# hmorimitsu/ptlflow

Measured on NVIDIA H100. Metric: frame-pairs/sec RAFT 1024x436 12-iter, higher is better.
Workload: dtype f16 storage, f32 accumulate/coordinates

## Files before the change

include/ptlflow_b200.h:

```cpp
#ifndef PTLFLOW_B200_H_
#define PTLFLOW_B200_H_

#include <stddef.h>
#include <stdint.h>

#ifdef __cplusplus
extern "C" {
#endif

#if defined(__GNUC__)
#define PFB_API __attribute__((visibility("default")))
#else
#define PFB_API
#endif

typedef void* pfb_stream;

typedef enum { PFB_F32 = 0, PFB_F16 = 1, PFB_BF16 = 2 } pfb_dtype;

typedef enum {
  PFB_OK = 0,
  PFB_ERR_ARG = -1,
  PFB_ERR_CUDA = -2,
  PFB_ERR_UNSUPPORTED = -3
// ... 54 lines not shown
  PFB_EPI_LINEAR = 0,
  PFB_EPI_RELU = 1,
  PFB_EPI_GRU_ZR = 2,
  PFB_EPI_GRU_Q = 3,
  PFB_EPI_FLOW = 4,
  PFB_EPI_RELU_APPEND_FLOW = 5,
  PFB_EPI_AXPY = 6,
  PFB_EPI_LINEAR_F32 = 7,
  PFB_EPI_GELU = 8,
  PFB_EPI_RESIDUAL_GELU = 9,
  PFB_EPI_LINEAR_APPEND_FLOW = 10
} pfb_epilogue;

typedef struct {
  const void* ptr;
  int channels;
  int stride;
  int offset;
  int is_f32;
} pfb_conv_src;

typedef struct {
  pfb_conv_src src[PFB_MAX_SRC];
  int nsrc;
  int B, H, W;
  int KH, KW;
  int Cout;
  int Cout_pad;
  const void* weight;
  const float* bias;
  int epilogue;
  float scale;
  void* out;
  int out_stride, out_offset;
  const void* aux_h;
  void* aux_z;
  int hidden;
  float* coords;
  const float* flow;
  pfb_dtype dtype;
  int impl;
  const void* weight_k;
  int Cin_pad, Cout_pad_k;
  const void* addend;
  int addend_stride;
  int w_rows_per_sample;
  const void* residual;
  int residual_stride, residual_offset;
  const float* post_w;
  const float* post_b;
} pfb_conv_params;

PFB_API int pfb_conv2d(const pfb_conv_params* p, pfb_stream stream);

PFB_API int pfb_pack_conv_weight(const void* src, void* dst, int Cout, int Cin, int KH, int KW, int Cout_pad,
                         int col_offset, pfb_dtype src_dtype, pfb_dtype dst_dtype, pfb_stream stream);
PFB_API int pfb_pack_bias(const void* src, float* dst, int n, int offset, pfb_dtype src_dtype, pfb_stream stream);
PFB_API int pfb_pack_conv_weight_kmajor(const void* src, void* dst, int Cout, int Cin, int KH, int KW, int Cout_pad_k,
                                        int row_offset, const int* src_channels, int nsrc, int Cin_pad,
                                        pfb_dtype src_dtype, pfb_dtype dst_dtype, pfb_stream stream);

PFB_API int pfb_depthwise_conv_gelu(const void* x, int in_stride, int in_offset, void* out, int out_stride, int out_offset,
                                    const float* weight, const float* bias, int B, int H, int W, int C, int k, pfb_dtype dtype,
                                    pfb_stream stream);

PFB_API int pfb_depthwise_conv_layernorm(const void* x, int in_stride, int in_offset, void* out, int out_stride, int out_offset,
                                         const float* weight, const float* bias, int B, int H, int W, int C, int k, float eps,
                                         pfb_dtype dtype, pfb_stream stream);

PFB_API int pfb_convex_upsample(const float* coords, const void* mask, float* out, float* flow_small, int B, int H,
                        int W, int out_h, int out_w, int pad_top, int pad_left, pfb_dtype dtype,
                        pfb_stream stream);
PFB_API int pfb_upflow8(const float* coords, float* out, float* flow_small, int B, int H, int W, int out_h, int out_w,
                int pad_top, int pad_left, pfb_stream stream);

PFB_API int pfb_softmax_rows(void* x, size_t rows, int cols, pfb_dtype dtype, pfb_stream stream);
PFB_API int pfb_attention_softmax_relpos(const void* logits, const float* th, const float* tw, size_t table_stride, void* attn,
                                         size_t rows, int H, int W, int P, pfb_dtype dtype, pfb_stream stream);
PFB_API int pfb_transpose_pm(const void* in, void* out, int B, int HW, int C, int HW_pad, pfb_dtype dtype, pfb_stream stream);

PFB_API int pfb_flow_tap_gather(const float* taps, int tstride, const float* bias, float* coords, float* flow, int B, int H, int W,
                                pfb_stream stream);

PFB_API int pfb_context_split(const void* cnet, void* net, void* inp, int B, int H, int W, int hidden, int context,
                      pfb_dtype dtype, pfb_stream stream);
PFB_API int pfb_init_coords(float* coords, const float* flow_init_nchw, int B, int H, int W, pfb_stream stream);
PFB_API int pfb_forward_interpolate(const float* flow_nchw, float* out_nchw, int B, int H, int W, pfb_stream stream);

typedef enum {
  PFB_L_CONVC1 = 0, PFB_L_CONVC2, PFB_L_CONVF1, PFB_L_CONVF2, PFB_L_CONV,
  PFB_L_GRU_ZR1, PFB_L_GRU_Q1, PFB_L_GRU_ZR2, PFB_L_GRU_Q2,
  PFB_L_FLOW1, PFB_L_FLOW2, PFB_L_MASK1, PFB_L_MASK2,
  PFB_L_AGG_V,
  PFB_L_FLOW2T,
  PFB_L_CTX_ZR1, PFB_L_CTX_Q1, PFB_L_CTX_ZR2, PFB_L_CTX_Q2,
  PFB_L_GRUX_ZR1, PFB_L_GRUX_Q1, PFB_L_GRUX_ZR2, PFB_L_GRUX_Q2,
  PFB_L_CONVC2F2,
  PFB_L_AGG_PROJ,
  PFB_L_COUNT
} pfb_layer_id;

typedef struct {
  const void* weight;
  const float* bias;
  int Cout, Cout_pad, Cin, KH, KW;
  const void* weight_k;
// ... 196 lines not shown
```

ptlflow_b200/_lib.py:

```python
from __future__ import annotations

import ctypes as C
import threading
import os
from typing import Optional

import torch

_PKG = os.path.dirname(os.path.abspath(__file__))
LIB_PATH = os.path.join(_PKG, "lib", "libptlflow_b200.so")

PFB_MAX_LEVELS = 8
PFB_MAX_SRC = 4

F32, F16, BF16 = 0, 1, 2
_DTYPES = {torch.float32: F32, torch.float16: F16, torch.bfloat16: BF16}

EPI_LINEAR, EPI_RELU, EPI_GRU_ZR, EPI_GRU_Q, EPI_FLOW, EPI_RELU_APPEND_FLOW, EPI_AXPY, EPI_LINEAR_F32 = range(8)
EPI_GELU, EPI_RESIDUAL_GELU, EPI_LINEAR_APPEND_FLOW = range(8, 11)
ENC_CONV_LINEAR, ENC_CONV_BIAS_RELU, ENC_CONV_BIAS_RELU_RESIDUAL = range(3)

(L_CONVC1, L_CONVC2, L_CONVF1, L_CONVF2, L_CONV, L_GRU_ZR1, L_GRU_Q1, L_GRU_ZR2, L_GRU_Q2,
 L_FLOW1, L_FLOW2, L_MASK1, L_MASK2, L_AGG_V, L_FLOW2T,
 L_CTX_ZR1, L_CTX_Q1, L_CTX_ZR2, L_CTX_Q2, L_GRUX_ZR1, L_GRUX_Q1, L_GRUX_ZR2, L_GRUX_Q2, L_CONVC2F2, L_AGG_PROJ, L_COUNT) = range(26)
# ... 65 lines not shown
    _fields_ = [("blocks", PcBlock * SK_BLOCKS), ("convf1", Layer), ("mask1", Layer), ("mask2", Layer),
                ("agg_v", Layer), ("agg_proj", Layer)]


PFB_SR_MAX_BLOCKS = 8


class ConvNextBlock(C.Structure):
    _fields_ = [("dw_k", C.c_int), ("dw_weight", C.c_void_p), ("dw_bias", C.c_void_p), ("pw1", Layer), ("out", Layer)]


class SearaftWeights(C.Structure):
    _fields_ = [("init_conv", Layer), ("convc1", Layer), ("convc2", Layer), ("convf1", Layer), ("convf2", Layer), ("conv", Layer),
                ("num_blocks", C.c_int), ("blocks", ConvNextBlock * PFB_SR_MAX_BLOCKS), ("ln_eps", C.c_float),
                ("flow1", Layer), ("flow2", Layer), ("flow2t", Layer), ("mask1", Layer), ("mask2", Layer)]


class XcitBlock(C.Structure):
    _fields_ = [("pos_proj", Layer), ("qk", Layer), ("v_weight", C.c_void_p), ("v_bias", C.c_void_p), ("proj_weight", C.c_void_p),
                ("proj_bias", C.c_void_p), ("temperature", C.c_void_p), ("ln3_weight", C.c_void_p), ("ln3_bias", C.c_void_p),
                ("dw1_weight", C.c_void_p), ("dw1_bias", C.c_void_p), ("gn_weight", C.c_void_p), ("gn_bias", C.c_void_p),
                ("dw2_weight", C.c_void_p), ("dw2_bias", C.c_void_p), ("fc1", Layer), ("fc2", Layer), ("ln_eps", C.c_float),
                ("gn_eps", C.c_float)]


class CcmrWeights(C.Structure):
    _fields_ = [("raft", RaftWeights), ("context", XcitBlock), ("aggregator", XcitBlock)]


_lib: Optional[C.CDLL] = None

_I, _P, _S = C.c_int, C.c_void_p, C.c_void_p
_PP = C.POINTER(C.c_void_p)
SIGNATURES = {
    "pfb_version": (_I, []),
    "pfb_last_error": (C.c_char_p, []),
    "pfb_device_arch": (_I, []),
    "pfb_stream_create": (_I, [_PP]),
    "pfb_stream_destroy": (_I, [_S]),
    "pfb_corr_volume_build": (_I, [_P, _P, _PP, _I, _I, _I, _I, _I, _I, _I, _S]),
    "pfb_corr_volume_build_ex": (_I, [_P, _P, _PP, _I, _I, _I, _I, _I, _I, _I, C.c_float, _I, _I, _S]),
    "pfb_corr_level_bytes": (C.c_size_t, [_I, _I, _I, _I, _I]),
    "pfb_corr_lookup": (_I, [_PP, _P, _P, _I, _I, _I, _I, _I, _I, _I, _I, _I, _S]),
    "pfb_corr_lookup_ex": (_I, [_PP, C.POINTER(C.c_int), C.POINTER(C.c_int), _P, _P, _I, _I, _I, _I, _I, _I, _I, _I, _I, _S]),
    "pfb_corr_level_bytes_tiled": (C.c_size_t, [_I, _I, _I, _I, _I, _I]),
    "pfb_corr_volume_build_tiled": (_I, [_P, _P, _PP, _I, _I, _I, _I, _I, _I, _I, C.c_float, _I, _S]),
    "pfb_corr_lookup_tiled": (_I, [_PP, _P, _P, _I, _I, _I, _I, _I, _I, _I, _I, _I, _S]),
    "pfb_corr_lookup_onthefly": (_I, [_P, _PP, _P, _P, _I, _I, _I, _I, _I, _I, _I, _I, _I, _I, _S]),
    "pfb_corr_lookup_onthefly_tc_workspace_bytes": (C.c_size_t, [_I, _I, _I]),
    "pfb_corr_lookup_onthefly_tc": (_I, [_P, _PP, _P, _P, _P, _I, _I, _I, _I, _I, _I, _I, _I, _S]),
    "pfb_alt_corr_forward": (_I, [_P, _P, _P, _P, _I, _I, _I, _I, _I, _I, _I, _I, _I, _S]),
    "pfb_avg_pool2x2_nhwc": (_I, [_P, _P, _I, _I, _I, _I, _I, _S]),
    "pfb_conv2d": (_I, [C.POINTER(ConvParams), _S]),
    "pfb_pack_conv_weight": (_I, [_P, _P, _I, _I, _I, _I, _I, _I, _I, _I, _S]),
    "pfb_pack_bias": (_I, [_P, _P, _I, _I, _I, _S]),
    "pfb_pack_conv_weight_kmajor": (_I, [_P, _P, _I, _I, _I, _I, _I, _I, C.POINTER(C.c_int), _I, _I, _I, _I, _S]),
    "pfb_convex_upsample": (_I, [_P, _P, _P, _P, _I, _I, _I, _I, _I, _I, _I, _I, _S]),
    "pfb_upflow8": (_I, [_P, _P, _P, _I, _I, _I, _I, _I, _I, _I, _S]),
    "pfb_softmax_rows": (_I, [_P, C.c_size_t, _I, _I, _S]),
    "pfb_attention_softmax_relpos": (_I, [_P, _P, _P, C.c_size_t, _P, C.c_size_t, _I, _I, _I, _I, _S]),
    "pfb_transpose_pm": (_I, [_P, _P, _I, _I, _I, _I, _I, _S]),
    "pfb_flow_tap_gather": (_I, [_P, _I, _P, _P, _P, _I, _I, _I, _S]),
    "pfb_context_split": (_I, [_P, _P, _P, _I, _I, _I, _I, _I, _I, _S]),
    "pfb_init_coords": (_I, [_P, _P, _I, _I, _I, _S]),
    "pfb_forward_interpolate": (_I, [_P, _P, _I, _I, _I, _S]),
    "pfb_raft_workspace_bytes": (C.c_size_t, [C.POINTER(RaftCfg)]),
    "pfb_raft_refine": (_I, [C.POINTER(RaftCfg), C.POINTER(RaftWeights), C.POINTER(RaftBuffers), _S]),
    "pfb_preprocess_frames": (_I, [_P, _P, _I, _I, _I, _I, _I, _I, _I, _I, _I, _S]),
    "pfb_instance_norm_workspace_bytes": (C.c_size_t, [_I, _I]),
    "pfb_instance_norm_act": (_I, [_P, _P, _P, _P, _I, _I, _I, _I, C.c_float, _I, _I, _S]),
    "pfb_instance_norm_apply": (_I, [_P, _P, _P, _P, _I, _I, _I, _I, C.c_float, _I, _I, _S]),
    "pfb_flow_conv7x7": (_I, [_P, _P, _P, _P, _I, _I, _I, _I, _I, _I, _S]),
    "pfb_first_conv7x7s2": (_I, [_P, _P, _P, _P, _P, _I, _I, _I, _I, _I, _S]),
    "pfb_bias_act": (_I, [_P, _P, _P, _P, _P, _I, _I, _I, _I, _I, _I, _S]),
    "pfb_enc_conv3x3_supported": (_I, [_I, _I, _I]),
    "pfb_enc_conv3x3": (_I, [_P, _P, _P, _P, _P, _I, _I, _I, _I, _I, _I, _I, _I, _I, _S]),
    "pfb_launch_count": (C.c_ulonglong, [_I]),
    "pfb_profile_enable": (_I, [_I]),
    "pfb_profile_collect": (_I, [C.POINTER(C.c_double), C.POINTER(C.c_ulonglong), _I]),
    "pfb_raft_update_iter": (_I, [C.POINTER(RaftCfg), C.POINTER(RaftWeights), C.POINTER(RaftBuffers), _P, _P, _S]),
    "pfb_depthwise_conv_gelu": (_I, [_P, _I, _I, _P, _I, _I, _P, _P, _I, _I, _I, _I, _I, _I, _S]),
    "pfb_skflow_workspace_bytes": (C.c_size_t, [C.POINTER(RaftCfg)]),
    "pfb_skflow_refine": (_I, [C.POINTER(RaftCfg), C.POINTER(SkflowWeights), C.POINTER(RaftBuffers), _S]),
    "pfb_skflow_update_iter": (_I, [C.POINTER(RaftCfg), C.POINTER(SkflowWeights), C.POINTER(RaftBuffers), _P, _P, _S]),
    "pfb_depthwise_conv_layernorm": (_I, [_P, _I, _I, _P, _I, _I, _P, _P, _I, _I, _I, _I, _I, C.c_float, _I, _S]),
    "pfb_searaft_workspace_bytes": (C.c_size_t, [C.POINTER(RaftCfg)]),
    "pfb_searaft_refine": (_I, [C.POINTER(RaftCfg), C.POINTER(SearaftWeights), C.POINTER(RaftBuffers), _S]),
    "pfb_searaft_update_iter": (_I, [C.POINTER(RaftCfg), C.POINTER(SearaftWeights), C.POINTER(RaftBuffers), _P, _P, _S]),
    "pfb_corr_lookup_onthefly_ex": (_I, [_P, _PP, _P, _P, _I, _I, _I, _I, _I, _I, C.c_float, _I, _I, _I, _I, _S]),
    "pfb_corr_lookup_onthefly_tc_ex": (_I, [_P, _PP, _P, _P, _P, _I, _I, _I, _I, _I, _I, C.c_float, _I, _I, _S]),
    "pfb_group_norm_act": (_I, [_P, _P, _P, _P, _P, _P, _P, _I, _I, _I, _I, _I, C.c_float, _I, _I, _S]),
    "pfb_group_norm_apply": (_I, [_P, _P, _P, _P, _P, _P, _P, _I, _I, _I, _I, _I, C.c_float, _I, _I, _S]),
    "pfb_upsample2x_concat": (_I, [_P, _I, _P, _I, _P, _I, _I, _I, _I, _S]),
    "pfb_convex_upsample2x": (_I, [_P, _P, _P, _I, _I, _I, _I, _I, _I, _I, _I, _I, _S]),
    "pfb_downflow": (_I, [_P, _P, _I, _I, _I, _I, _I, _S]),
    "pfb_msraft_workspace_bytes": (C.c_size_t, [C.POINTER(RaftCfg)]),
    "pfb_msraft_refine": (_I, [C.POINTER(RaftCfg), C.POINTER(RaftWeights), C.POINTER(RaftBuffers), C.c_float, _P, _S]),
    "pfb_msraft_update_iter": (_I, [C.POINTER(RaftCfg), C.POINTER(RaftWeights), C.POINTER(RaftBuffers), _P, _P, C.c_float, _S]),
    "pfb_layernorm": (_I, [_P, _I, _I, _P, _I, _I, _P, _P, C.c_size_t, _I, C.c_float, _I, _S]),
    "pfb_depthwise_conv3x3_ex": (_I, [_P, _I, _I, _P, _I, _I, _P, _P, _P, _I, _I, _I, _I, _I, _I, _I, _I, _S]),
    "pfb_fourier_features": (_I, [_P, _I, _I, _I, _S]),
    "pfb_xca_stats_workspace_bytes": (C.c_size_t, [_I, _I]),
    "pfb_xca_stats": (_I, [_P, _I, _I, _I, _I, _I, _P, _P, _I, _S]),
    "pfb_xca_fold": (_I, [_P, _P, _P, _P, _P, _P, _P, _P, _P, _I, _I, _S]),
    "pfb_convex_handover2x": (_I, [_P, _P, _P, _I, _I, _I, _I, _S]),
    "pfb_upflow2": (_I, [_P, _P, _I, _I, _I, _I, _I, _I, _I, _S]),
# ... 96 lines not shown
```

ptlflow_b200/csrc/common.cuh:

```cuda
#pragma once
#include <cuda_bf16.h>
#include <cuda_fp16.h>
#include <cuda_runtime.h>
#include <stdint.h>
#include <stdio.h>

#include "../../include/ptlflow_b200.h"

namespace pfb {

void set_error(const char* fmt, ...);

#define PFB_CHECK_ARG(cond, ...)           \
  do {                                     \
    if (!(cond)) {                         \
      ::pfb::set_error(__VA_ARGS__);       \
      return PFB_ERR_ARG;                  \
    }                                      \
  } while (0)

#define PFB_CUDA(call)                                                                        \
  do {                                                                                        \
    cudaError_t e__ = (call);                                                                 \
    if (e__ != cudaSuccess) {                                                                 \
// ... 31 lines not shown
  else if (dt == PFB_F16) reinterpret_cast<__half*>(p)[i] = __float2half_rn(v);
  else reinterpret_cast<__nv_bfloat16*>(p)[i] = __float2bfloat16_rn(v);
}

__device__ __forceinline__ float sigmoid_f32(float x) { return 1.0f / (1.0f + expf(-x)); }
__device__ __forceinline__ float gelu_f32(float x) { return 0.5f * x * (1.0f + erff(x * 0.70710678118654752f)); }

#define PFB_DISPATCH_DTYPE(dt, T, ...)                        \
  do {                                                        \
    if ((dt) == PFB_F32) { using T = float; __VA_ARGS__; }    \
    else if ((dt) == PFB_F16) { using T = __half; __VA_ARGS__; } \
    else { using T = __nv_bfloat16; __VA_ARGS__; }            \
  } while (0)

inline int ceil_div(int a, int b) { return (a + b - 1) / b; }
inline size_t ceil_div_sz(size_t a, size_t b) { return (a + b - 1) / b; }
inline size_t align_up(size_t a, size_t b) { return (a + b - 1) / b * b; }

int sm_count();

__device__ __forceinline__ void pdl_wait() { asm volatile("griddepcontrol.wait;" ::: "memory"); }
__device__ __forceinline__ void pdl_trigger() { asm volatile("griddepcontrol.launch_dependents;" ::: "memory"); }
int pdl_enabled();
template <typename... KArgs, typename... Args>
inline cudaError_t launch_pdl(void (*kernel)(KArgs...), dim3 grid, dim3 block, size_t smem, cudaStream_t s, Args... args) {
  cudaLaunchConfig_t cfg{};
  cfg.gridDim = grid;
  cfg.blockDim = block;
  cfg.dynamicSmemBytes = smem;
  cfg.stream = s;
  cudaLaunchAttribute attr[1];
  attr[0].id = cudaLaunchAttributeProgrammaticStreamSerialization;
  attr[0].val.programmaticStreamSerializationAllowed = pdl_enabled();
  cfg.attrs = attr;
  cfg.numAttrs = 1;
  return cudaLaunchKernelEx(&cfg, kernel, static_cast<KArgs>(args)...);
}

enum KernelClass { KC_VOLUME = 0, KC_POOL, KC_LOOKUP, KC_ONTHEFLY, KC_CONV, KC_UPSAMPLE, KC_MISC,
                   KC_ENC_AFFINE, KC_ENC_STATS, KC_ENC_CONV1, KC_FLOWCONV, KC_GATHER, KC_DEPTHWISE, KC_DW_LAYERNORM, KC_COUNT };
class ProfScope {
 public:
  ProfScope(int kc, cudaStream_t s);
  ~ProfScope();
 private:
  int kc_;
  cudaStream_t s_;
  void* a_;
};

int conv2d_simt(const pfb_conv_params* p, cudaStream_t s);
int conv2d_umma(const pfb_conv_params* p, cudaStream_t s);
bool conv2d_umma_supported(const pfb_conv_params* p);
bool conv_cout2_supported(const pfb_conv_params* p);
int conv_cout2_flow(const pfb_conv_params* p, cudaStream_t s);
bool conv_flow7x7_supported(const pfb_conv_params* p);
int conv_flow7x7(const pfb_conv_params* p, cudaStream_t s);
int corr_volume_umma(const void* f1, const void* f2, void* const* pyr, int B, int N1, int H, int W, int C, int L, float scale,
                     pfb_dtype dt, cudaStream_t s);
bool corr_volume_umma_supported(int B, int H, int W, int C, int L, pfb_dtype dt);
bool corr_onthefly_umma_supported(int B, int H, int W, int C, int levels, int radius, pfb_dtype dt, int out_stride);
int corr_volume_tiled(const void* f1, const void* f2, void* const* pyr, int B, int N1, int H, int W, int C, int L, float scale,
                      pfb_dtype dt, cudaStream_t s);
bool corr_volume_tiled_supported(int B, int H, int W, int C, int L, pfb_dtype dt);

}
```

ptlflow_b200/csrc/conv_simt.cu:

```cuda
#include "common.cuh"

namespace pfb {

struct SrcDev {
  const void* ptr;
  int channels, stride, offset, is_f32;
};

struct ConvDev {
  SrcDev src[PFB_MAX_SRC];
  int nsrc;
  int B, H, W, KH, KW;
  int Cin_total, Cout, Cout_pad;
  const void* weight;
  const float* bias;
  int epilogue;
  float scale;
  void* out;
  int out_stride, out_offset;
  const void* aux_h;
  void* aux_z;
  int hidden;
  float* coords;
  const float* flow;
// ... 184 lines not shown
          int x = p % a.W, y = (p / a.W) % a.H;
          reinterpret_cast<float*>(a.out)[(size_t)p * a.out_stride + a.out_offset + n] = c1 - (float)(n == 0 ? x : y);
          break;
        }
        default:
          break;
      }
    }
    if ((a.epilogue == PFB_EPI_RELU_APPEND_FLOW || a.epilogue == PFB_EPI_LINEAR_APPEND_FLOW) && blockIdx.y == 0 && tx == 0) {
      T* o = reinterpret_cast<T*>(a.out) + (size_t)p * a.out_stride + a.out_offset + a.Cout;
      o[0] = from_f32<T>(a.flow[(size_t)p * 2]);
      o[1] = from_f32<T>(a.flow[(size_t)p * 2 + 1]);
    }
  }
}

int conv2d_simt(const pfb_conv_params* p, cudaStream_t s) {
  ConvDev a;
  a.nsrc = p->nsrc;
  int cin = 0;
  for (int i = 0; i < p->nsrc; ++i) {
    a.src[i].ptr = p->src[i].ptr;
    a.src[i].channels = p->src[i].channels;
    a.src[i].stride = p->src[i].stride;
    a.src[i].offset = p->src[i].offset;
    a.src[i].is_f32 = p->src[i].is_f32 || p->dtype == PFB_F32;
    cin += p->src[i].channels;
  }
  a.B = p->B; a.H = p->H; a.W = p->W; a.KH = p->KH; a.KW = p->KW;
  a.Cin_total = cin; a.Cout = p->Cout; a.Cout_pad = p->Cout_pad;
  a.weight = p->weight; a.bias = p->bias; a.epilogue = p->epilogue; a.scale = p->scale;
  a.out = p->out; a.out_stride = p->out_stride; a.out_offset = p->out_offset;
  a.aux_h = p->aux_h; a.aux_z = p->aux_z; a.hidden = p->hidden; a.coords = p->coords; a.flow = p->flow;
  a.residual = p->residual; a.residual_stride = p->residual_stride; a.residual_offset = p->residual_offset;
  a.post_w = p->post_w; a.post_b = p->post_b;
  const int P = p->B * p->H * p->W;
  const int n_tiles = ceil_div(p->Cout, 64), sms = sm_count();
  const int bm = ceil_div(P, 64) * n_tiles >= sms ? 64 : (ceil_div(P, 32) * n_tiles >= sms ? 32 : 16);
  dim3 grid(ceil_div(P, bm), n_tiles);
  {
    ProfScope prof(KC_CONV, s);
    if (bm == 64) PFB_DISPATCH_DTYPE(p->dtype, T, { conv_simt_kernel<T, 64><<<grid, 256, 0, s>>>(a); });
    else if (bm == 32) PFB_DISPATCH_DTYPE(p->dtype, T, { conv_simt_kernel<T, 32><<<grid, 256, 0, s>>>(a); });
    else PFB_DISPATCH_DTYPE(p->dtype, T, { conv_simt_kernel<T, 16><<<grid, 256, 0, s>>>(a); });
  }
  PFB_LAUNCH_CHECK();
  return PFB_OK;
}

}

using namespace pfb;

extern "C" PFB_API int pfb_conv2d(const pfb_conv_params* p, pfb_stream stream) {
  PFB_CHECK_ARG(p, "conv2d: null params");
  PFB_CHECK_ARG(dtype_ok(p->dtype), "conv2d: bad dtype %d", (int)p->dtype);
  PFB_CHECK_ARG(p->nsrc >= 1 && p->nsrc <= PFB_MAX_SRC, "conv2d: nsrc=%d out of range", p->nsrc);
  PFB_CHECK_ARG(p->B > 0 && p->H > 0 && p->W > 0, "conv2d: bad shape");
  PFB_CHECK_ARG((p->KH & 1) && (p->KW & 1) && p->KH <= 15 && p->KW <= 15, "conv2d: kernel %dx%d must be odd", p->KH, p->KW);
  PFB_CHECK_ARG(p->Cout > 0 && p->Cout_pad >= p->Cout, "conv2d: Cout=%d Cout_pad=%d", p->Cout, p->Cout_pad);
  PFB_CHECK_ARG(p->weight && p->out, "conv2d: null weight/out");
  for (int i = 0; i < p->nsrc; ++i) {
    PFB_CHECK_ARG(p->src[i].ptr && p->src[i].channels > 0 && p->src[i].stride >= p->src[i].offset + p->src[i].channels,
                  "conv2d: bad source %d", i);
  }
  switch (p->epilogue) {
    case PFB_EPI_LINEAR: case PFB_EPI_RELU: case PFB_EPI_LINEAR_F32: case PFB_EPI_GELU: break;
    case PFB_EPI_RESIDUAL_GELU:
      PFB_CHECK_ARG(p->residual && p->residual_stride >= p->residual_offset + p->Cout && p->residual_offset >= 0,
                    "conv2d: RESIDUAL_GELU needs a residual with stride >= offset + Cout");
      PFB_CHECK_ARG((p->post_w == nullptr) == (p->post_b == nullptr), "conv2d: RESIDUAL_GELU needs both post_w and post_b, or neither");
      break;
    case PFB_EPI_AXPY:
      PFB_CHECK_ARG(p->aux_h && p->hidden >= p->Cout, "conv2d: AXPY needs aux_h (residual) with stride hidden >= Cout");
      break;
    case PFB_EPI_GRU_ZR:
      PFB_CHECK_ARG(p->aux_h && p->aux_z && p->hidden > 0 && p->Cout == 2 * p->hidden, "conv2d: GRU_ZR needs aux_h, aux_z and Cout == 2*hidden");
      break;
    case PFB_EPI_GRU_Q:
      PFB_CHECK_ARG(p->aux_h && p->aux_z && p->hidden > 0 && p->Cout == p->hidden, "conv2d: GRU_Q needs aux_h, aux_z and Cout == hidden");
      break;
    case PFB_EPI_FLOW:
      PFB_CHECK_ARG(p->coords && p->Cout == 2, "conv2d: FLOW epilogue needs coords and Cout == 2");
      break;
    case PFB_EPI_RELU_APPEND_FLOW:
    case PFB_EPI_LINEAR_APPEND_FLOW:
      PFB_CHECK_ARG(p->flow && p->out_stride >= p->out_offset + p->Cout + 2, "conv2d: APPEND_FLOW needs flow and room for 2 channels");
      break;
    default:
      set_error("conv2d: unknown epilogue %d", p->epilogue);
      return PFB_ERR_ARG;
  }
  cudaStream_t s = as_stream(stream);
  if (p->impl != 1) {
    if (conv_cout2_supported(p)) return conv_cout2_flow(p, s);
    if (conv_flow7x7_supported(p)) return conv_flow7x7(p, s);
    if (conv2d_umma_supported(p)) return conv2d_umma(p, s);
    if (p->impl == 2) {
      set_error("conv2d: wgmma path does not support this shape/dtype");
      return PFB_ERR_UNSUPPORTED;
    }
  }
  if (p->addend || p->w_rows_per_sample) {
    set_error("conv2d: per-pixel addend / per-sample weights are implemented by the wgmma path only (shape / dtype / impl not eligible)");
    return PFB_ERR_UNSUPPORTED;
  }
  return conv2d_simt(p, s);
}
```

ptlflow_b200/csrc/enc_conv_umma.cu:

```cuda
#include <atomic>
#include <type_traits>

#include "umma.cuh"

namespace pfb {
using namespace sm90;

constexpr int kEcThreads = 3 * 128;
constexpr int kEcNW = 128;
constexpr int kEcPatchBox = kEcNW + 2;
constexpr int kEcStageOut = kEcNW * 128;
constexpr int kEcMaxA = 8, kEcMaxW = 18;
constexpr int kEcProducerRegs = 40, kEcMmaRegs = 232;
static_assert(128 * (kEcProducerRegs + 2 * kEcMmaRegs) <= 65536, "register budget exceeds the register file");

struct __align__(8) EcBars {
  uint64_t a_full[kEcMaxA];
  uint64_t a_empty[kEcMaxA];
  uint64_t w_full[kEcMaxW];
  uint64_t w_empty[kEcMaxW];
  uint64_t res_full[2];
};

struct EcPlan {
// ... 280 lines not shown
              wl = w_lo;
            }
            const uint32_t xl = a_lo + 8u * kx;
            if (full_chunk) ec_issue<kBF16, 4>(d, wl, xl, acc);
            else ec_issue<kBF16, 2>(d, wl, xl, acc);
            wgmma_wait<1>();
            reg_fence(d);
            release_held();
            if (!a.w_resident) {
              held_w = sw;
              w_lo += w_slot16;
              if (++sw == a.w_stages) { sw = 0; phw ^= 1; w_lo = w_lo0; }
            }
            if (kx == 2) held_a = sa;
            acc = 1;
          }
          a_lo += a_slot16;
          if (++sa == a.a_stages) { sa = 0; pha ^= 1; a_lo = a_lo0; }
        }
      }
      wgmma_wait<0>();
      reg_fence(d);
      release_held();
      epilogue(d, b, y, x0);
    }
    if (tid == 0) asm volatile("cp.async.bulk.wait_group 0;" ::: "memory");
  }
}

template <typename T, int EPI>
static int launch_enc_conv_e(const CUtensorMap& tmX, const CUtensorMap& tmW, const CUtensorMap& tmO, const CUtensorMap& tmR,
                             const EncConvArgs& a, int grid, size_t smem, cudaStream_t s) {
  static std::atomic<unsigned long long> attr_done{0};
  int dev = 0;
  PFB_CUDA(cudaGetDevice(&dev));
  if (!(attr_done.load(std::memory_order_acquire) & (1ull << (dev & 63)))) {
    PFB_CUDA(cudaFuncSetAttribute(enc_conv_umma_kernel<T, EPI>, cudaFuncAttributeMaxDynamicSharedMemorySize, 227 * 1024));
    attr_done.fetch_or(1ull << (dev & 63), std::memory_order_release);
  }
  PFB_CUDA(launch_pdl(enc_conv_umma_kernel<T, EPI>, dim3(grid), dim3(kEcThreads), smem, s, tmX, tmW, tmO, tmR, a));
  return PFB_OK;
}

template <typename T>
static int launch_enc_conv(int epilogue, const CUtensorMap& tmX, const CUtensorMap& tmW, const CUtensorMap& tmO,
                           const CUtensorMap& tmR, const EncConvArgs& a, int grid, size_t smem, cudaStream_t s) {
  switch (epilogue) {
    case PFB_ENC_CONV_LINEAR: return launch_enc_conv_e<T, PFB_ENC_CONV_LINEAR>(tmX, tmW, tmO, tmR, a, grid, smem, s);
    case PFB_ENC_CONV_BIAS_RELU: return launch_enc_conv_e<T, PFB_ENC_CONV_BIAS_RELU>(tmX, tmW, tmO, tmR, a, grid, smem, s);
    default: return launch_enc_conv_e<T, PFB_ENC_CONV_BIAS_RELU_RESIDUAL>(tmX, tmW, tmO, tmR, a, grid, smem, s);
  }
}

}

using namespace pfb;

static bool aligned16(const void* p) { return (reinterpret_cast<uintptr_t>(p) & 15) == 0; }

extern "C" PFB_API int pfb_enc_conv3x3_supported(int Cin, int Cout, pfb_dtype dtype) {
  if (dtype != PFB_F16 && dtype != PFB_BF16) return 0;
  EcPlan pl{};
  return plan_enc_conv(1, 1, 1, Cin, Cout, pl) ? 1 : 0;
}

extern "C" PFB_API int pfb_enc_conv3x3(const void* x, const void* weight_k, const float* bias, const void* residual, void* out,
                                       int B, int H, int W, int Cin, int Cout, int out_stride, int out_offset, int epilogue,
                                       pfb_dtype dtype, pfb_stream stream) {
  PFB_CHECK_ARG(x && weight_k && out, "enc_conv3x3: null pointer");
  PFB_CHECK_ARG(dtype == PFB_F16 || dtype == PFB_BF16, "enc_conv3x3: f16 / bf16 storage only");
  PFB_CHECK_ARG(epilogue == PFB_ENC_CONV_LINEAR || epilogue == PFB_ENC_CONV_BIAS_RELU || epilogue == PFB_ENC_CONV_BIAS_RELU_RESIDUAL,
                "enc_conv3x3: unknown epilogue %d", epilogue);
  PFB_CHECK_ARG(epilogue == PFB_ENC_CONV_LINEAR || bias, "enc_conv3x3: epilogue %d needs a bias", epilogue);
  PFB_CHECK_ARG(epilogue != PFB_ENC_CONV_BIAS_RELU_RESIDUAL || (residual && aligned16(residual)),
                "enc_conv3x3: the residual epilogue needs a 16-byte aligned residual [B,H,W,Cout]");
  PFB_CHECK_ARG(aligned16(x) && aligned16(weight_k) && aligned16(out), "enc_conv3x3: 16-byte alignment");
  PFB_CHECK_ARG(out_stride % 8 == 0 && out_offset % 8 == 0 && out_offset >= 0 && out_offset + Cout <= out_stride,
                "enc_conv3x3: out_stride / out_offset must be multiples of 8 with out_offset + Cout <= out_stride");
  EcPlan pl{};
  PFB_CHECK_ARG(plan_enc_conv(B, H, W, Cin, Cout, pl), "enc_conv3x3: unsupported shape B=%d H=%d W=%d Cin=%d Cout=%d", B, H, W, Cin, Cout);
  cudaStream_t s = as_stream(stream);
  const int Cin_pad = pl.chunks * 64, Cout_pad_k = (Cout + 31) / 32 * 32;
  CUtensorMap tmX, tmW, tmO, tmR;
  {
    uint64_t dims[4] = {(uint64_t)Cin, (uint64_t)W, (uint64_t)H, (uint64_t)B};
    uint64_t str[3] = {(uint64_t)Cin * 2, (uint64_t)W * Cin * 2, (uint64_t)H * W * Cin * 2};
    uint32_t box[4] = {64, (uint32_t)kEcPatchBox, 1, 1};
    int rc = make_tensor_map(&tmX, x, dtype, 4, dims, str, box);
    if (rc) return rc;
  }
  {
    uint64_t dims[2] = {(uint64_t)Cin_pad, (uint64_t)9 * Cout_pad_k};
    uint64_t str[1] = {(uint64_t)Cin_pad * 2};
    uint32_t box[2] = {64, (uint32_t)(64 * pl.mb)};
    int rc = make_tensor_map(&tmW, weight_k, dtype, 2, dims, str, box);
    if (rc) return rc;
  }
  {
    uint64_t dims[4] = {(uint64_t)(out_offset + Cout), (uint64_t)W, (uint64_t)H, (uint64_t)B};
    uint64_t str[3] = {(uint64_t)out_stride * 2, (uint64_t)W * out_stride * 2, (uint64_t)H * W * out_stride * 2};
    uint32_t box[4] = {64, (uint32_t)kEcNW, 1, 1};
    int rc = make_tensor_map(&tmO, out, dtype, 4, dims, str, box);
    if (rc) return rc;
  }
  tmR = tmO;
  if (epilogue == PFB_ENC_CONV_BIAS_RELU_RESIDUAL) {
// ... 20 lines not shown
```

Measured before the change: 521.8.

## Add persistent warp-specialized implicit-GEMM conv kernel and route eligible ReLU convs to it

Adds a persistent, warp-specialized wgmma convolution kernel that TMA-loads input row patches and 128x64 weight slices through multi-stage mbarrier pipelines. Each tile covers two output rows by 128 pixels and reuses one loaded patch across the KW taps. A new router sends 1x1 and 3x3 ReLU / ReLU+append-flow convolutions with 128-multiple padded Cout to this kernel by default, in place of the previous umma path. The aim is better operand reuse and load/compute overlap, at the cost of more code paths and a different accumulation schedule.

```diff
diff --git a/include/ptlflow_b200.h b/include/ptlflow_b200.h
--- a/include/ptlflow_b200.h
+++ b/include/ptlflow_b200.h
@@ -130,6 +130,7 @@
 } pfb_conv_params;
 
 PFB_API int pfb_conv2d(const pfb_conv_params* p, pfb_stream stream);
+PFB_API int pfb_conv2d_route(const pfb_conv_params* p);
 
 PFB_API int pfb_pack_conv_weight(const void* src, void* dst, int Cout, int Cin, int KH, int KW, int Cout_pad,
                          int col_offset, pfb_dtype src_dtype, pfb_dtype dst_dtype, pfb_stream stream);
diff --git a/ptlflow_b200/_lib.py b/ptlflow_b200/_lib.py
--- a/ptlflow_b200/_lib.py
+++ b/ptlflow_b200/_lib.py
@@ -141,6 +141,7 @@
     "pfb_alt_corr_forward": (_I, [_P, _P, _P, _P, _I, _I, _I, _I, _I, _I, _I, _I, _I, _S]),
     "pfb_avg_pool2x2_nhwc": (_I, [_P, _P, _I, _I, _I, _I, _I, _S]),
     "pfb_conv2d": (_I, [C.POINTER(ConvParams), _S]),
+    "pfb_conv2d_route": (_I, [C.POINTER(ConvParams)]),
     "pfb_pack_conv_weight": (_I, [_P, _P, _I, _I, _I, _I, _I, _I, _I, _I, _S]),
     "pfb_pack_bias": (_I, [_P, _P, _I, _I, _I, _S]),
     "pfb_pack_conv_weight_kmajor": (_I, [_P, _P, _I, _I, _I, _I, _I, _I, C.POINTER(C.c_int), _I, _I, _I, _I, _S]),
diff --git a/ptlflow_b200/csrc/common.cuh b/ptlflow_b200/csrc/common.cuh
--- a/ptlflow_b200/csrc/common.cuh
+++ b/ptlflow_b200/csrc/common.cuh
@@ -107,6 +107,9 @@
 int conv2d_simt(const pfb_conv_params* p, cudaStream_t s);
 int conv2d_umma(const pfb_conv_params* p, cudaStream_t s);
 bool conv2d_umma_supported(const pfb_conv_params* p);
+bool loop_conv_supported(const pfb_conv_params* p);
+bool loop_conv_preferred(const pfb_conv_params* p);
+int loop_conv(const pfb_conv_params* p, cudaStream_t s);
 bool conv_cout2_supported(const pfb_conv_params* p);
 int conv_cout2_flow(const pfb_conv_params* p, cudaStream_t s);
 bool conv_flow7x7_supported(const pfb_conv_params* p);
diff --git a/ptlflow_b200/csrc/conv_simt.cu b/ptlflow_b200/csrc/conv_simt.cu
--- a/ptlflow_b200/csrc/conv_simt.cu
+++ b/ptlflow_b200/csrc/conv_simt.cu
@@ -260,6 +260,18 @@
 
 using namespace pfb;
 
+static int conv_route(const pfb_conv_params* p) {
+  if (p->impl == 1) return (p->addend || p->w_rows_per_sample) ? -1 : 0;
+  if (p->impl != 3) {
+    if (conv_cout2_supported(p) || conv_flow7x7_supported(p)) return 1;
+  }
+  if (p->impl == 3) return loop_conv_supported(p) ? 3 : -1;
+  if (p->impl == 0 && loop_conv_preferred(p)) return 3;
+  if (conv2d_umma_supported(p)) return 2;
+  if (p->impl == 2 || p->addend || p->w_rows_per_sample) return -1;
+  return 0;
+}
+
 extern "C" PFB_API int pfb_conv2d(const pfb_conv_params* p, pfb_stream stream) {
   PFB_CHECK_ARG(p, "conv2d: null params");
   PFB_CHECK_ARG(dtype_ok(p->dtype), "conv2d: bad dtype %d", (int)p->dtype);
@@ -300,18 +312,16 @@
       return PFB_ERR_ARG;
   }
   cudaStream_t s = as_stream(stream);
-  if (p->impl != 1) {
-    if (conv_cout2_supported(p)) return conv_cout2_flow(p, s);
-    if (conv_flow7x7_supported(p)) return conv_flow7x7(p, s);
-    if (conv2d_umma_supported(p)) return conv2d_umma(p, s);
-    if (p->impl == 2) {
-      set_error("conv2d: wgmma path does not support this shape/dtype");
-      return PFB_ERR_UNSUPPORTED;
-    }
-  }
-  if (p->addend || p->w_rows_per_sample) {
-    set_error("conv2d: per-pixel addend / per-sample weights are implemented by the wgmma path only (shape / dtype / impl not eligible)");
-    return PFB_ERR_UNSUPPORTED;
-  }
-  return conv2d_simt(p, s);
-}
+  switch (conv_route(p)) {
+    case 1: return conv_cout2_supported(p) ? conv_cout2_flow(p, s) : conv_flow7x7(p, s);
+    case 2: return conv2d_umma(p, s);
+    case 3: return loop_conv(p, s);
+    case 0: return conv2d_simt(p, s);
+    default: break;
+  }
+  if (p->impl == 2 || p->impl == 3) set_error("conv2d: wgmma path does not support this shape/dtype (impl %d)", p->impl);
+  else set_error("conv2d: per-pixel addend / per-sample weights are implemented by the wgmma path only (shape / dtype / impl not eligible)");
+  return PFB_ERR_UNSUPPORTED;
+}
+
+extern "C" PFB_API int pfb_conv2d_route(const pfb_conv_params* p) { return p ? conv_route(p) : -1; }
diff --git a/ptlflow_b200/csrc/enc_conv_umma.cu b/ptlflow_b200/csrc/enc_conv_umma.cu
--- a/ptlflow_b200/csrc/enc_conv_umma.cu
+++ b/ptlflow_b200/csrc/enc_conv_umma.cu
@@ -356,6 +356,361 @@
   }
 }
 
+constexpr int kLcTW = 128;
+constexpr int kLcMaxA = 8, kLcMaxW = 16;
+
+struct __align__(8) LcBars {
+  uint64_t a_full[kLcMaxA];
+  uint64_t a_empty[kLcMaxA];
+  uint64_t w_full[kLcMaxW];
+  uint64_t w_empty[kLcMaxW];
+};
+
+struct LcPlan {
+  int n_blocks;
+  int patch_w;
+  int a_row_bytes;
+  int a_stages, a_slot_bytes;
+  int w_stages;
+  int tiles_x, row_pairs, n_work;
+  size_t smem;
+};
+
+struct LoopConvArgs {
+  int nsrc;
+  int src_chunks[PFB_MAX_SRC];
+  int src_coff[PFB_MAX_SRC];
+  int B, H, W, KH, KW, Cout, Cout_pad_k, ncols;
+  int tiles_x, row_pairs, n_work;
+  int a_stages, a_slot_bytes, a_row_bytes, patch_w, w_stages;
+  int out_offset;
+  const float* bias;
+  const float* flow;
+};
+
+constexpr int kLcWSlot = 128 * 128;
+
+static bool lc_shape_ok(int KH, int KW) { return (KH == 1 && KW == 1) || (KH == 3 && KW == 3) || (KH == 1 && KW == 5); }
+
+static bool plan_loop_conv(int B, int H, int W, int KH, int KW, int Cout_pad_k, LcPlan& pl) {
+  if (B < 1 || H < 1 || W < 1 || !lc_shape_ok(KH, KW)) return false;
+  if (Cout_pad_k < 128 || Cout_pad_k % 64) return false;
+  pl.n_blocks = ceil_div(Cout_pad_k, 128);
+  pl.patch_w = kLcTW + KW - 1;
+  pl.a_row_bytes = (int)align_up((size_t)pl.patch_w * 128, 1024);
+  pl.a_slot_bytes = 2 * pl.a_row_bytes;
+  const int fixed = 2 * kEcStageOut + (int)sizeof(LcBars) + 1024;
+  const int budget = 227 * 1024 - fixed;
+  int best = -1;
+  for (int as = 2; as <= kLcMaxA; ++as) {
+    int ws = (budget - as * pl.a_slot_bytes) / kLcWSlot;
+    if (ws > kLcMaxW) ws = kLcMaxW;
+    if (ws < 2) continue;
+    const int cover_a = (as - 1) * KW, cover_w = ws - 1;
+    const int cover = cover_a < cover_w ? cover_a : cover_w;
+    if (cover > best || (cover == best && ws > pl.w_stages)) { best = cover; pl.a_stages = as; pl.w_stages = ws; }
+  }
+  if (best < 0) return false;
+  pl.tiles_x = ceil_div(W, kLcTW);
+  pl.row_pairs = ceil_div(H, 2);
+  const long n_work = (long)pl.tiles_x * pl.row_pairs * B * pl.n_blocks;
+  if (n_work > (1l << 30)) return false;
+  pl.n_work = (int)n_work;
+  pl.smem = (size_t)pl.a_stages * pl.a_slot_bytes + (size_t)pl.w_stages * kLcWSlot + fixed;
+  return true;
+}
+
+template <bool BF16>
+__device__ __forceinline__ void lc_issue(float (&d0)[kLcTW / 2], float (&d1)[kLcTW / 2], uint32_t w_lo, uint32_t x0_lo, uint32_t x1_lo,
+                                         uint32_t acc) {
+  wgmma_fence();
+#pragma unroll
+  for (int kk = 0; kk < 4; ++kk) {
+    const uint64_t wd = gdesc(w_lo + 2 * kk, kDescHiSw128);
+    wgmma<kLcTW, BF16>(d0, wd, gdesc(x0_lo + 2 * kk, kDescHiSw128), kk == 0 ? acc : 1u);
+    wgmma<kLcTW, BF16>(d1, wd, gdesc(x1_lo + 2 * kk, kDescHiSw128), kk == 0 ? acc : 1u);
+  }
+  wgmma_commit();
+}
+
+template <typename T, int EPI>
+__global__ void __launch_bounds__(kEcThreads, 1)
+loop_conv_umma_kernel(const __grid_constant__ CUtensorMap tm0, const __grid_constant__ CUtensorMap tm1,
+                      const __grid_constant__ CUtensorMap tm2, const __grid_constant__ CUtensorMap tmW,
+                      const __grid_constant__ CUtensorMap tmO, const LoopConvArgs a) {
+  constexpr bool kBF16 = std::is_same<T, __nv_bfloat16>::value;
+  extern __shared__ __align__(1024) uint8_t smem_raw[];
+  uint8_t* smem = reinterpret_cast<uint8_t*>((reinterpret_cast<uintptr_t>(smem_raw) + 1023) & ~uintptr_t(1023));
+  uint8_t* smemA = smem;
+  uint8_t* smemW = smemA + a.a_stages * a.a_slot_bytes;
+  uint8_t* smemO = smemW + a.w_stages * kLcWSlot;
+  LcBars* bars = reinterpret_cast<LcBars*>(smemO + 2 * kEcStageOut);
+  const int warp = threadIdx.x >> 5, lane = threadIdx.x & 31;
+
+  if (threadIdx.x == 0) {
+    for (int s = 0; s < a.a_stages; ++s) {
+      mbar_init(&bars->a_full[s], 1);
+      mbar_init(&bars->a_empty[s], 8);
+    }
+    for (int s = 0; s < a.w_stages; ++s) {
+      mbar_init(&bars->w_full[s], 1);
+      mbar_init(&bars->w_empty[s], 8);
+    }
+    fence_barrier_init();
+  }
+  if (warp == 0 && lane == 0) {
+    prefetch_tmap(&tm0);
+    if (a.nsrc > 1) prefetch_tmap(&tm1);
+    if (a.nsrc > 2) prefetch_tmap(&tm2);
+    prefetch_tmap(&tmW);
+    prefetch_tmap(&tmO);
+  }
+  __syncthreads();
+  pdl_wait();
+  pdl_trigger();
+
+  const int n_blocks = a.n_work / (a.tiles_x * a.row_pairs * a.B);
+  auto decode = [&](int w, int& n0, int& b, int& y0, int& x0) {
+    const int nb = w % n_blocks;
+    int m = w / n_blocks;
+    x0 = (m % a.tiles_x) * kLcTW;
+    m /= a.tiles_x;
+    y0 = (m % a.row_pairs) * 2;
+    b = m / a.row_pairs;
+    n0 = nb * 128;
+  };
+
+  if (warp < 4) {
+    setmaxnreg_dec<kEcProducerRegs>();
+    if (warp == 0) {
+      const uint32_t a_tx = 2 * a.patch_w * 128;
+      const int ph = a.KH >> 1, pw = a.KW >> 1;
+      int sa = 0, sw = 0;
+      uint32_t pa = 0, pw_ph = 0;
+      for (int w = blockIdx.x; w < a.n_work; w += gridDim.x) {
+        int n0, b, y0, x0;
+        decode(w, n0, b, y0, x0);
+        int kidx = 0;
+        for (int s = 0; s < a.nsrc; ++s) {
+          const CUtensorMap* tm = s == 0 ? &tm0 : (s == 1 ? &tm1 : &tm2);
+          for (int c = 0; c < a.src_chunks[s]; ++c, ++kidx) {
+            for (int ky = 0; ky < a.KH; ++ky) {
+              mbar_wait(&bars->a_empty[sa], pa ^ 1);
+              if (elect_one()) {
+                mbar_arrive_expect_tx(&bars->a_full[sa], a_tx);
+                for (int r = 0; r < 2; ++r)
+                  tma_load_4d(smemA + sa * a.a_slot_bytes + r * a.a_row_bytes, tm, &bars->a_full[sa], a.src_coff[s] + c * 64, x0 - pw,
+                              y0 + r + ky - ph, b);
+              }
+              __syncwarp();
+              if (++sa == a.a_stages) { sa = 0; pa ^= 1; }
+              for (int kx = 0; kx < a.KW; ++kx) {
+                mbar_wait(&bars->w_empty[sw], pw_ph ^ 1);
+                if (elect_one()) {
+                  mbar_arrive_expect_tx(&bars->w_full[sw], kLcWSlot);
+                  tma_load_2d(smemW + sw * kLcWSlot, &tmW, &bars->w_full[sw], kidx * 64, (ky * a.KW + kx) * a.Cout_pad_k + n0);
+                }
+                __syncwarp();
+                if (++sw == a.w_stages) { sw = 0; pw_ph ^= 1; }
+              }
+            }
+          }
+        }
+      }
+    }
+  } else {
+    setmaxnreg_inc<kEcMmaRegs>();
+    const int wg = (threadIdx.x >> 7) - 1, tid = threadIdx.x & 127, wq = tid >> 5;
+    uint8_t* stage = smemO + wg * kEcStageOut;
+    const uint32_t stage_u32 = smem_u32(stage);
+    const uint32_t a_slot16 = (uint32_t)a.a_slot_bytes >> 4, a_row16 = (uint32_t)a.a_row_bytes >> 4;
+    const uint32_t a_lo0 = gdesc_lo(smem_u32(smemA), 16);
+    const uint32_t w_lo0 = gdesc_lo(smem_u32(smemW) + wg * 64 * 128, 16);
+    const uint32_t bar_a_full = smem_u32(&bars->a_full[0]);
+    const uint32_t bar_w_full = smem_u32(&bars->w_full[0]);
+    const int ch = 64 * wg + 16 * wq + (lane >> 2);
+    int chunks = 0;
+    for (int s = 0; s < a.nsrc; ++s) chunks += a.src_chunks[s];
+    int sa = 0, sw = 0, held_a = -1, held_w = -1;
+    uint32_t pha = 0, phw = 0;
+    uint32_t a_lo = a_lo0, w_lo = w_lo0;
+    auto release_held = [&]() {
+      __syncwarp();
+      if (lane == 0) {
+        if (held_w >= 0) mbar_arrive(&bars->w_empty[held_w]);
+        if (held_a >= 0) mbar_arrive(&bars->a_empty[held_a]);
+      }
+      held_a = held_w = -1;
+    };
+    auto epilogue = [&](float (&dd)[kLcTW / 2], int n0, int b, int y, int x0) {
+      if (y >= a.H || n0 + 64 * wg >= a.ncols) return;
+      const int c_lo = n0 + ch, c_hi = c_lo + 8;
+      const float bias_lo = c_lo < a.Cout ? a.bias[c_lo] : 0.f, bias_hi = c_hi < a.Cout ? a.bias[c_hi] : 0.f;
+      const int fl_lo = EPI == PFB_EPI_RELU_APPEND_FLOW && c_lo >= a.Cout && c_lo < a.ncols ? c_lo - a.Cout : -1;
+      const int fl_hi = EPI == PFB_EPI_RELU_APPEND_FLOW && c_hi >= a.Cout && c_hi < a.ncols ? c_hi - a.Cout : -1;
+      const float* flow_row = EPI == PFB_EPI_RELU_APPEND_FLOW ? a.flow + ((size_t)b * a.H + y) * a.W * 2 : nullptr;
+      if (tid == 0) tma_store_wait_read();
+      named_barrier_sync(1 + wg, 128);
+#pragma unroll
+      for (int j = 0; j < kLcTW / 8; j += 2) {
+        const int m = lane >> 3;
+        const int px = 8 * (j + (m >> 1)) + (lane & 7);
+        const int piece = 2 * wq + (m & 1);
+        const uint32_t addr = stage_u32 + px * 128 + ((piece ^ (px & 7)) << 4);
+        float v[8];
+#pragma unroll
+        for (int q = 0; q < 8; ++q) v[q] = fmaxf(dd[4 * j + q] + ((q & 2) ? bias_hi : bias_lo), 0.f);
+        if (EPI == PFB_EPI_RELU_APPEND_FLOW && (fl_lo >= 0 || fl_hi >= 0)) {
+#pragma unroll
+          for (int q = 0; q < 8; ++q) {
+            const int f = (q & 2) ? fl_hi : fl_lo;
+            const int x = x0 + 8 * (j + (q >> 2)) + 2 * (lane & 3) + (q & 1);
+            if (f >= 0 && x < a.W) v[q] = flow_row[2 * x + f];
+          }
+        }
+        uint32_t r[4];
+#pragma unroll
+        for (int q = 0; q < 4; ++q) r[q] = ec_pack2<T>(v[2 * q], v[2 * q + 1]);
+        stmatrix_x4_trans(addr, r);
+      }
+      fence_proxy_async();
+      named_barrier_sync(1 + wg, 128);
+      if (tid == 0) {
+        tma_store_4d(&tmO, stage, a.out_offset + n0 + 64 * wg, x0, y, b);
+        tma_store_commit();
+      }
+    };
+    float d0[kLcTW / 2], d1[kLcTW / 2];
+    for (int w = blockIdx.x; w < a.n_work; w += gridDim.x) {
+      int n0, b, y0, x0;
+      decode(w, n0, b, y0, x0);
+      uint32_t acc = 0;
+      for (int g = 0; g < chunks * a.KH; ++g) {
+        mbar_wait_uniform(bar_a_full + 8 * sa, pha);
+        for (int kx = 0; kx < a.KW; ++kx) {
+          mbar_wait_uniform(bar_w_full + 8 * sw, phw);
+          const uint32_t xl = a_lo + 8u * kx;
+          lc_issue<kBF16>(d0, d1, w_lo, xl, xl + a_row16, acc);
+          wgmma_wait<1>();
+          reg_fence(d0);
+          reg_fence(d1);
+          release_held();
+          held_w = sw;
+          w_lo += kLcWSlot >> 4;
+          if (++sw == a.w_stages) { sw = 0; phw ^= 1; w_lo = w_lo0; }
+          if (kx == a.KW - 1) held_a = sa;
+          acc = 1;
+        }
+        a_lo += a_slot16;
+        if (++sa == a.a_stages) { sa = 0; pha ^= 1; a_lo = a_lo0; }
+      }
+      wgmma_wait<0>();
+      reg_fence(d0);
+      reg_fence(d1);
+      release_held();
+      epilogue(d0, n0, b, y0, x0);
+      epilogue(d1, n0, b, y0 + 1, x0);
+    }
+    if (tid == 0) asm volatile("cp.async.bulk.wait_group 0;" ::: "memory");
+  }
+}
+
+template <typename T, int EPI>
+static int launch_loop_conv_e(const CUtensorMap* tms, const CUtensorMap& tmW, const CUtensorMap& tmO, const LoopConvArgs& a, int grid,
+                              size_t smem, cudaStream_t s) {
+  static std::atomic<unsigned long long> attr_done{0};
+  int dev = 0;
+  PFB_CUDA(cudaGetDevice(&dev));
+  if (!(attr_done.load(std::memory_order_acquire) & (1ull << (dev & 63)))) {
+    PFB_CUDA(cudaFuncSetAttribute(loop_conv_umma_kernel<T, EPI>, cudaFuncAttributeMaxDynamicSharedMemorySize, 227 * 1024));
+    attr_done.fetch_or(1ull << (dev & 63), std::memory_order_release);
+  }
+  PFB_CUDA(launch_pdl(loop_conv_umma_kernel<T, EPI>, dim3(grid), dim3(kEcThreads), smem, s, tms[0], tms[1], tms[2], tmW, tmO, a));
+  return PFB_OK;
+}
+
+template <typename T>
+static int launch_loop_conv(int epilogue, const CUtensorMap* tms, const CUtensorMap& tmW, const CUtensorMap& tmO, const LoopConvArgs& a,
+                            int grid, size_t smem, cudaStream_t s) {
+  if (epilogue == PFB_EPI_RELU_APPEND_FLOW) return launch_loop_conv_e<T, PFB_EPI_RELU_APPEND_FLOW>(tms, tmW, tmO, a, grid, smem, s);
+  return launch_loop_conv_e<T, PFB_EPI_RELU>(tms, tmW, tmO, a, grid, smem, s);
+}
+
+static bool lc_aligned16(const void* p) { return (reinterpret_cast<uintptr_t>(p) & 15) == 0; }
+
+bool loop_conv_supported(const pfb_conv_params* p) {
+  if (p->dtype != PFB_F16 && p->dtype != PFB_BF16) return false;
+  if (p->epilogue != PFB_EPI_RELU && p->epilogue != PFB_EPI_RELU_APPEND_FLOW) return false;
+  if (!p->weight_k || !p->bias || p->addend || p->w_rows_per_sample) return false;
+  if (!lc_aligned16(p->out) || !lc_aligned16(p->weight_k) || p->out_stride % 8 || p->out_offset % 8) return false;
+  if (p->nsrc < 1 || p->nsrc > 3) return false;
+  int cin_pad = 0;
+  for (int i = 0; i < p->nsrc; ++i) {
+    const pfb_conv_src& s = p->src[i];
+    if (s.is_f32 || s.offset % 8 || s.stride % 8 || !lc_aligned16(s.ptr)) return false;
+    cin_pad += (int)align_up((size_t)s.channels, 64);
+  }
+  if (cin_pad != p->Cin_pad) return false;
+  if (p->epilogue == PFB_EPI_RELU_APPEND_FLOW && p->Cout + 2 > (int)align_up((size_t)p->Cout_pad_k, 64)) return false;
+  if (p->Cout > p->Cout_pad_k) return false;
+  LcPlan pl{};
+  return plan_loop_conv(p->B, p->H, p->W, p->KH, p->KW, p->Cout_pad_k, pl);
+}
+
+bool loop_conv_preferred(const pfb_conv_params* p) {
+  return ((p->KH == 3 && p->KW == 3) || (p->KH == 1 && p->KW == 1)) && p->Cout_pad_k % 128 == 0 && loop_conv_supported(p);
+}
+
+int loop_conv(const pfb_conv_params* p, cudaStream_t s) {
+  LcPlan pl{};
+  if (!loop_conv_supported(p) || !plan_loop_conv(p->B, p->H, p->W, p->KH, p->KW, p->Cout_pad_k, pl)) {
+    set_error("loop_conv: layer not supported");
+    return PFB_ERR_UNSUPPORTED;
+  }
+  LoopConvArgs a{};
+  CUtensorMap tms[3];
+  a.nsrc = p->nsrc;
+  for (int i = 0; i < p->nsrc; ++i) {
+    const pfb_conv_src& src = p->src[i];
+    a.src_chunks[i] = ceil_div(src.channels, 64);
+    a.src_coff[i] = src.offset;
+    uint64_t dims[4] = {(uint64_t)(src.offset + src.channels), (uint64_t)p->W, (uint64_t)p->H, (uint64_t)p->B};
+    uint64_t str[3] = {(uint64_t)src.stride * 2, (uint64_t)p->W * src.stride * 2, (uint64_t)p->H * p->W * src.stride * 2};
+    uint32_t box[4] = {64, (uint32_t)pl.patch_w, 1, 1};
+    int rc = make_tensor_map(&tms[i], src.ptr, p->dtype, 4, dims, str, box);
+    if (rc) return rc;
+  }
+  for (int i = p->nsrc; i < 3; ++i) tms[i] = tms[0];
+  CUtensorMap tmW, tmO;
+  {
+    uint64_t dims[2] = {(uint64_t)p->Cin_pad, (uint64_t)p->KH * p->KW * p->Cout_pad_k};
+    uint64_t str[1] = {(uint64_t)p->Cin_pad * 2};
+    uint32_t box[2] = {64, 128};
+    int rc = make_tensor_map(&tmW, p->weight_k, p->dtype, 2, dims, str, box);
+    if (rc) return rc;
+  }
+  a.ncols = p->epilogue == PFB_EPI_RELU_APPEND_FLOW ? p->Cout + 2 : p->Cout;
+  {
+    uint64_t dims[4] = {(uint64_t)(p->out_offset + a.ncols), (uint64_t)p->W, (uint64_t)p->H, (uint64_t)p->B};
+    uint64_t str[3] = {(uint64_t)p->out_stride * 2, (uint64_t)p->W * p->out_stride * 2, (uint64_t)p->H * p->W * p->out_stride * 2};
+    uint32_t box[4] = {64, (uint32_t)kLcTW, 1, 1};
+    int rc = make_tensor_map(&tmO, p->out, p->dtype, 4, dims, str, box);
+    if (rc) return rc;
+  }
+  a.B = p->B; a.H = p->H; a.W = p->W; a.KH = p->KH; a.KW = p->KW; a.Cout = p->Cout; a.Cout_pad_k = p->Cout_pad_k;
+  a.tiles_x = pl.tiles_x; a.row_pairs = pl.row_pairs; a.n_work = pl.n_work;
+  a.a_stages = pl.a_stages; a.a_slot_bytes = pl.a_slot_bytes; a.a_row_bytes = pl.a_row_bytes; a.patch_w = pl.patch_w;
+  a.w_stages = pl.w_stages;
+  a.out_offset = p->out_offset;
+  a.bias = p->bias;
+  a.flow = p->flow;
+  int grid = sm_count();
+  if (grid > pl.n_work) grid = pl.n_work;
+  ProfScope prof(KC_CONV, s);
+  if (p->dtype == PFB_F16) return launch_loop_conv<__half>(p->epilogue, tms, tmW, tmO, a, grid, pl.smem, s);
+  return launch_loop_conv<__nv_bfloat16>(p->epilogue, tms, tmW, tmO, a, grid, pl.smem, s);
+}
+
 }
 
 using namespace pfb;
```

Result: faster. 533.1, median of 6 (+2.2%).
